# Tianion/topazdb

Hardware: AMD Instinct MI355X
Metric: GiB/s device-resident SSTable block decode+checksum, 4KiB blocks, 1 MI355X (higher is better)
Workload: dtype u8; 1 GPU; 4k: 1048576 blocks/GPU x 4155 B median, 34.0 entries/block, tag 1 (Uncompress); blocks_per_gpu=1048576, input_bytes_per_gpu=4356833280, parallelism=shard1

## Files before the change

### topazdb_amd/csrc/tpz_decode.hip

```cpp

#include <hip/hip_runtime.h>
#include <stdint.h>

#include "tpz_internal.h"
#include "tpz_spill.hip"

namespace tpz {

typedef uint32_t u32;
typedef uint64_t u64;

constexpr int kWave = 64;
#ifdef TPZ_ABL_W20
#ifdef TPZ_ABL_W8
constexpr int kWavesPerWG = 8;
#else
constexpr int kWavesPerWG = 10;
#endif
#else
constexpr int kWavesPerWG = 16;
#endif
constexpr int kWGThreads = kWave * kWavesPerWG;
constexpr u32 kRowShift = 4, kRowBlocks = 1u << kRowShift;
#ifndef TPZ_ROW_AHEAD
#define TPZ_ROW_AHEAD 3
#endif
constexpr u32 kRowAhead = TPZ_ROW_AHEAD, kRowRing = 16;
constexpr u32 kRowExit = 0xFFFFFFFFu;
constexpr int kTableBytes = kNumCrcTables * 256 * 4;
constexpr int kGuard = 96;

constexpr int kWinRounds = 5;
constexpr int kWinBytes = 4352;
constexpr u32 kWaveMaxLen = kWinBytes - 16;
#ifdef TPZ_ABL_W20
constexpr int kWaveTabBytes = 16 * 1024;
constexpr u32 kWaveMaxN = 63;
constexpr int kWaveTabSlots = 128;
#else
constexpr int kWaveTabBytes = kTableBytes;
constexpr u32 kWaveMaxN = 255;
constexpr int kWaveTabSlots = 512;
#endif
constexpr int kWaveMapLen = 288;
constexpr int kSlotBytes = kGuard + kWinBytes + 32 + kWaveTabSlots * 4 + 2 * kWaveMapLen;
static_assert(kSlotBytes % 16 == 0 && kWaveMapLen % 8 == 0, "slot alignment");
static_assert(2 * kWaveMaxN + 1 <= (u32)kWaveTabSlots, "entry table");
constexpr int kWaveLds = kWaveTabBytes + kWavesPerWG * kSlotBytes;
static_assert(kWaveLds <= 163840, "wave path LDS");

constexpr int kBigWaves = 16;
constexpr int kBigThreads = kBigWaves * kWave;
constexpr int kBigWinBytes = 94208;
constexpr u32 kBigMaxLen = TPZ_LDS_BLOCK_BYTES;
constexpr int kBigMapLen = 5904;
constexpr int kBigStage = (kBigWinBytes + 16 * kBigThreads - 1) / (16 * kBigThreads);
constexpr int kBigMaxGroups = 736;
constexpr int kBigMaxWin = 96;
constexpr int kBigLdsSlots = 960;
constexpr int kBigSuper = 20;
constexpr int kBigLds = kTableBytes + kGuard + kBigWinBytes + 32 + kBigMapLen * 2 +
                        kBigMaxGroups * 10 + kBigMaxWin * 4 + kBigWaves * 4 + kBigLdsSlots * 8;
static_assert(kBigMaxLen + 16 <= kBigWinBytes, "big window");
static_assert(kBigMapLen % 8 == 0 && (kWaveMaxLen + 2) / 16 + 3 <= (u32)kWaveMapLen &&
              (kBigMaxLen + 2) / 16 + 3 <= (u32)kBigMapLen, "map sizes");
static_assert(kBigLds <= 163840, "big path LDS");
static_assert((kTableBytes + kGuard + kBigWinBytes + 32 + kBigMapLen * 2 + kBigMaxWin * 4 +
               kBigWaves * 4) % 8 == 0, "big path entry table alignment");

__device__ __forceinline__ u32 lane_id() {
  u32 l = __builtin_amdgcn_mbcnt_hi(~0u, __builtin_amdgcn_mbcnt_lo(~0u, 0u));
  asm volatile("" : "+v"(l));
  return l;
}
__device__ __forceinline__ u32 uni(u32 x) { return __builtin_amdgcn_readfirstlane(x); }
__device__ __forceinline__ u64 uni64(u64 x) {
  u32 lo = __builtin_amdgcn_readfirstlane((u32)x), hi = __builtin_amdgcn_readfirstlane((u32)(x >> 32));
  return ((u64)hi << 32) | lo;
}
__device__ __forceinline__ u32 readlane(u32 x, int l) { return __builtin_amdgcn_readlane(x, l); }
template <int CTRL>
__device__ __forceinline__ u32 dpp(u32 x) {
  return (u32)__builtin_amdgcn_update_dpp(0, (int)x, CTRL, 0xF, 0xF, true);
}
constexpr int kRowShr = 0x110;
constexpr int kRowShl = 0x100;

__device__ __forceinline__ u32 lds_u32(const uint8_t* base, u32 a) {
  const u32* p = reinterpret_cast<const u32*>(base + (a & ~3u));
  return __builtin_amdgcn_alignbyte(p[1], p[0], a & 3u);
}
__device__ __forceinline__ u32 lds_be16(const uint8_t* base, u32 a) {
  u32 w = lds_u32(base, a);
  return ((w & 0xFFu) << 8) | ((w >> 8) & 0xFFu);
}
__device__ __forceinline__ u32 bswap32(u32 w) { return __builtin_bswap32(w); }

__device__ __forceinline__ uint4 lds_window16(const uint8_t* base, int x) {
  typedef u32 u32x2 __attribute__((ext_vector_type(2)));
  const u32x2* p = reinterpret_cast<const u32x2*>(base + (x & ~7));
  u32x2 a = p[0], b = p[1], c = p[2];
  asm volatile("" : "+v"(a), "+v"(b), "+v"(c));
  const u32 s = (u32)x & 3u;
  const bool h = ((u32)x & 4u) != 0;
  const u32 s0 = h ? a.y : a.x, s1 = h ? b.x : a.y, s2 = h ? b.y : b.x, s3 = h ? c.x : b.y,
            s4 = h ? c.y : c.x;
  return make_uint4(__builtin_amdgcn_alignbyte(s1, s0, s), __builtin_amdgcn_alignbyte(s2, s1, s),
                    __builtin_amdgcn_alignbyte(s3, s2, s), __builtin_amdgcn_alignbyte(s4, s3, s));
}

#ifdef TPZ_ABL_NOCF
__device__ __forceinline__ u32 tlook(const u32* tab, int id, u32 byte) {
  u32 z = byte;
  asm volatile("" : "+v"(z));
  return tab[id * 256 + (((z & 0x10000u) + __builtin_amdgcn_mbcnt_lo(~0u, 0u)) & 31u)];
}
#elif defined(TPZ_ABL_W20)
__device__ __forceinline__ u32 tlook(const u32* tab, int id, u32 byte) { return tab[(id & 15) * 256 + byte]; }
#else
__device__ __forceinline__ u32 tlook(const u32* tab, int id, u32 byte) { return tab[id * 256 + byte]; }
#endif

__device__ __forceinline__ u32 xor3(u32 a, u32 b, u32 c) { return __builtin_amdgcn_bitop3_b32(a, b, c, 0x96); }

__device__ __forceinline__ u32 slice16(const u32* tab, u32 w0, u32 w1, u32 w2, u32 w3) {
  u32 c = xor3(tlook(tab, 15, w0 & 0xFF), tlook(tab, 14, (w0 >> 8) & 0xFF), tlook(tab, 13, (w0 >> 16) & 0xFF));
  c = xor3(c, tlook(tab, 12, w0 >> 24), tlook(tab, 11, w1 & 0xFF));
  c = xor3(c, tlook(tab, 10, (w1 >> 8) & 0xFF), tlook(tab, 9, (w1 >> 16) & 0xFF));
  c = xor3(c, tlook(tab, 8, w1 >> 24), tlook(tab, 7, w2 & 0xFF));
  c = xor3(c, tlook(tab, 6, (w2 >> 8) & 0xFF), tlook(tab, 5, (w2 >> 16) & 0xFF));
  c = xor3(c, tlook(tab, 4, w2 >> 24), tlook(tab, 3, w3 & 0xFF));
  c = xor3(c, tlook(tab, 2, (w3 >> 8) & 0xFF), tlook(tab, 1, (w3 >> 16) & 0xFF));
  return c ^ tlook(tab, 0, w3 >> 24);
}

__device__ __forceinline__ u32 crc_shift_small(const u32* tab, u32 a, u32 k) {
  u32 r = k >= 4 ? 0u : (a >> (8 * k));
  for (u32 i = 0; i < 4 && i < k; i++) r ^= tlook(tab, (int)(k - 1 - i), (a >> (8 * i)) & 0xFF);
  return r;
}

__device__ __forceinline__ u32 crc_unshift_small(const u32* tab, u32 r, u32 k) {
#ifdef TPZ_ABL_W20
  return r;
#endif
  for (u32 i = 0; i < k; i++) {
    const u32 b = tlook(tab, kCrcInvTable, r >> 24);
    r = ((r ^ tlook(tab, 0, b)) << 8) | b;
  }
  return r;
}

__device__ __forceinline__ u32 gf_mul(u32 a, u32 b) {
  u32 p = 0;
#pragma unroll
  for (int i = 0; i < 32; i++) {
    p ^= (a & (0x80000000u >> i)) ? b : 0u;
    b = (b >> 1) ^ ((b & 1u) ? 0xEDB88320u : 0u);
  }
  return p;
}

__device__ __forceinline__ u32 gf_mul_lane(u32 a, u32 b) {
  u32 p = 0;
#pragma unroll
  for (int i = 0; i < 32; i++) {
    const u32 m = (u32)((int)(a << i) >> 31);
    p ^= b & m;
    b = (b >> 1) ^ (0xEDB88320u & (u32)(-(int)(b & 1u)));
  }
  return p;
}

__device__ __forceinline__ u32 wave_xor(u32 x) {
  x ^= (u32)__builtin_amdgcn_update_dpp(0, (int)x, 0x100 + 1, 0xF, 0xF, true);
  x ^= (u32)__builtin_amdgcn_update_dpp(0, (int)x, 0x100 + 2, 0xF, 0xF, true);
  x ^= (u32)__builtin_amdgcn_update_dpp(0, (int)x, 0x100 + 4, 0xF, 0xF, true);
  x ^= (u32)__builtin_amdgcn_update_dpp(0, (int)x, 0x100 + 8, 0xF, 0xF, true);
  return __builtin_amdgcn_readlane(x, 0) ^ __builtin_amdgcn_readlane(x, 16) ^
         __builtin_amdgcn_readlane(x, 32) ^ __builtin_amdgcn_readlane(x, 48);
}

template <int J>
__device__ __forceinline__ u32 crc_shift(const u32* tab, u32 a) {
  constexpr int b0 = 16 + 4 * J;
  return xor3(tlook(tab, b0, a & 0xFF), tlook(tab, b0 + 1, (a >> 8) & 0xFF),
              tlook(tab, b0 + 2, (a >> 16) & 0xFF)) ^ tlook(tab, b0 + 3, a >> 24);
}

__device__ __forceinline__ uint4 keep_head(uint4 v, u32 k) {
  const u64 lo = (u64)v.y << 32 | v.x, hi = (u64)v.w << 32 | v.z;
  const u64 mlo = k >= 8 ? ~0ull : ((1ull << (8 * k)) - 1);
  const u64 mhi = k >= 16 ? ~0ull : (k <= 8 ? 0ull : ((1ull << (8 * (k - 8))) - 1));
  const u64 a = lo & mlo, b = hi & mhi;
  return make_uint4((u32)a, (u32)(a >> 32), (u32)b, (u32)(b >> 32));
}

__device__ __forceinline__ uint4 zero_head(uint4 v, u32 k) {
  const u64 lo = (u64)v.y << 32 | v.x, hi = (u64)v.w << 32 | v.z;
  const u64 mlo = k >= 8 ? 0ull : (~0ull << (8 * k));
// ... 487 lines not shown
    j++;
    e0 = e1, d0 = d1, e1 = e2, d1 = d2, e2 = e3, d2 = d3;
  }
  const bool b1 = act && j + 1 < F.nk && e0 < x0 + 16;
  const bool b2 = b1 && j + 2 < F.nk && e1 < x0 + 16;
  uint4 acc = src(act ? (int)x0 + d0 : -kGuard);
  const uint4 n1 = src(b1 ? (int)x0 + d1 : -kGuard);
  const uint4 n2 = src(b2 ? (int)x0 + d2 : -kGuard);
  const bool rw = __ballot(act && (e0 <= x0 || (b2 && e2 < x0 + 16 && j + 3 < F.nk))) != 0;
  if (rw) rare |= 1u << w;
  if (b1) acc = merge_at(acc, n1, (int)(e0 - x0));
  if (b2) acc = merge_at(acc, n2, (int)(e1 - x0));
  if (FLAT)
    D.put(c, acc, rw);
  else
    __builtin_amdgcn_raw_buffer_store_b128(__builtin_bit_cast(__attribute__((ext_vector_type(4))) u32, acc),
                                           F.out, rw ? kOob : x0, 0, 0);
  return carry_out;
}

template <bool SHORT, bool FLAT, class S>
__device__ __forceinline__ u32 copy_crc_fused(const u32* tab, const S& src, const ColSmall& col,
                                              const uint16_t* map, u32 nk, u32 tot, uint8_t* dst,
                                              const FlatOut& D, const uint8_t* win, int pb, u32 Pa,
                                              u32 kshift, Stamps& St, u32 w3, const Out& o,
                                              PendingCrc& pd) {
  const u32 lane = lane_id();
  FastWin F;
  F.nk = nk;
  F.tot = tot;
  F.nch = (tot + 15) >> 4;
  F.npad = FLAT ? F.nch : (F.nch + 7) & ~7u;
  F.last = nk ? nk - 1 : 0u;
  F.out = __builtin_amdgcn_make_buffer_rsrc(dst, (short)0, FLAT ? 0 : (int)(F.npad * 16), 0x00020000);
  const u32 nw = (F.npad + 63) >> 6;
  CrcLane L;
  L.seg = (int)Pa - kCrcLaneBytes * (int)(lane + 1);
  L.act = L.seg + kCrcLaneBytes > 0;
  L.c = 0;
  u32 carry = 0, rare = 0, cw[5];
  const bool pl = pd.live != 0;
  u32 cA = pd.lc, want = 0;
  CombLv cl{0u, 0u, 0u, 0u};
  if (pl) {
    cl = comb_issue<0>(tab, cA);
    want = crc_shift_small(tab, ~pd.stored, pd.k);
  }
#pragma unroll
  for (int t = 0; t < 4; t++) {
    cw[t] = carry;
    crc_step(tab, win, pb, L, t);
    carry = (SHORT && (u32)t < w3) ? copy_fast3<FLAT>(src, col, map, F, D, (u32)t, carry, rare)
                                   : copy_fast<FLAT>(src, col, map, F, D, (u32)t, carry, rare);
    if (pl) {
      if (t == 0) { cA = comb_use<0>(cA, cl); cl = comb_issue<1>(tab, cA); }
      if (t == 1) { cA = comb_use<1>(cA, cl); cl = comb_issue<2>(tab, cA); }
      if (t == 2) { cA = comb_use<2>(cA, cl); cl = comb_issue<3>(tab, cA); }
      if (t == 3) { cA = comb_use<3>(cA, cl); cl = comb_issue<4>(tab, cA); }
    }
  }
  cw[4] = carry;
  crc_step(tab, win, pb, L, 4);
  if (pl) {
    cA = comb_use<4>(cA, cl);
    cl = comb_issue<5>(tab, cA);
  }
  if (nw > 4)
    carry = (SHORT && 4u < w3) ? copy_fast3<FLAT>(src, col, map, F, D, 4u, carry, rare)
                               : copy_fast<FLAT>(src, col, map, F, D, 4u, carry, rare);
  if (pl) comb_finish(tab, o, pd, comb_use<5>(cA, cl), want);
  TPZ_STAMP(St, 4);
#ifdef TPZ_ABL_STAMPS
  St.rare += __builtin_popcount(rare);
#endif
  if (rare) {
    for (u32 w = 0; w < nw; w++)
      if (rare & (1u << w)) {
        if (FLAT)
          copy_window(src, col, map, nk, F.tot, FlatDst{&D}, (u32)kWaveMapLen, w, cw[w]);
        else
          copy_window(src, col, map, nk, F.tot, SlotDst{dst, F.npad, F.tot}, (u32)kWaveMapLen, w, cw[w]);
      }
  }
  return crc_lane_value(tab, L);
}

typedef u32 u32x2v __attribute__((ext_vector_type(2)));
typedef u32 u32x4v __attribute__((ext_vector_type(4)));
struct Gath {
  u32 d0, d1, d2, d3, d4;
};
__device__ __forceinline__ Gath gath_issue(const uint8_t* base, int x) {
  const u32* p = reinterpret_cast<const u32*>(base + (x & ~3));
  Gath g;
  g.d0 = p[0];
  g.d1 = p[1];
  g.d2 = p[2];
  g.d3 = p[3];
  g.d4 = p[4];
  return g;
}
__device__ __forceinline__ uint4 gath_finish(Gath g, int x) {
  asm volatile("" : "+v"(g.d0), "+v"(g.d1), "+v"(g.d2), "+v"(g.d3), "+v"(g.d4));
  const u32 s = (u32)x & 3u;
  return make_uint4(__builtin_amdgcn_alignbyte(g.d1, g.d0, s), __builtin_amdgcn_alignbyte(g.d2, g.d1, s),
                    __builtin_amdgcn_alignbyte(g.d3, g.d2, s), __builtin_amdgcn_alignbyte(g.d4, g.d3, s));
}
struct Look16 {
  u32 r[16];
};
__device__ __forceinline__ Look16 look_issue(const u32* tab, u32x4v w, u32 c) {
  Look16 L;
  const u32 w0 = w.x ^ c;
#pragma unroll
  for (int i = 0; i < 4; i++) {
    L.r[i] = tlook(tab, 15 - i, (w0 >> (8 * i)) & 0xFF);
    L.r[4 + i] = tlook(tab, 11 - i, (w.y >> (8 * i)) & 0xFF);
    L.r[8 + i] = tlook(tab, 7 - i, (w.z >> (8 * i)) & 0xFF);
    L.r[12 + i] = tlook(tab, 3 - i, (w.w >> (8 * i)) & 0xFF);
  }
  return L;
}
__device__ __forceinline__ u32 look_xor(const Look16& L) {
  u32 c = xor3(L.r[0], L.r[1], L.r[2]);
  c = xor3(c, L.r[3], L.r[4]);
  c = xor3(c, L.r[5], L.r[6]);
  c = xor3(c, L.r[7], L.r[8]);
  c = xor3(c, L.r[9], L.r[10]);
  c = xor3(c, L.r[11], L.r[12]);
  c = xor3(c, L.r[13], L.r[14]);
  return c ^ L.r[15];
}
#define TPZ_SB() __builtin_amdgcn_sched_barrier(0)

struct PWin {
  u32 m, j;
  u32 e0, e1;
  int d0, d1;
  bool act, cross;
  Gath ga, gn;
};
struct PWin3 {
  u32 e2, e3;
  int d2, d3;
  bool b2;
  Gath g2;
};

struct RegGeom {
  u32 n, KL, VL, db;
};
constexpr u32 kRegShift = 26;
__device__ __forceinline__ u32 reg_recip(u32 d) {
  u32 m = (u32)(__builtin_amdgcn_rcpf((float)d) * (float)(1u << kRegShift)) + 2u;
  asm volatile("" : "+v"(m));
  return uni(m);
}
__device__ __forceinline__ u32 mul24(u32 a, u32 b) { return (a & 0xFFFFFFu) * (b & 0xFFFFFFu); }
__device__ __forceinline__ u32 reg_div(u32 y, u32 m) {
  const u64 p = (u64)(y & 0x1FFFu) * (u64)(m & 0x7FFFFFu);
  return __builtin_amdgcn_alignbit((u32)(p >> 32), (u32)p, kRegShift) & 0x3FFu;
}

template <bool FLAT, u32 K3, bool REG = false>
__device__ __forceinline__ u32 copy_crc_piped(const u32* tab, const ColSmall& col,
                                              const uint16_t* map, u32 nk, u32 tot, uint8_t* dst,
                                              const FlatOut& D, const uint8_t* win, int pb, u32 Pa,
                                              const Out& o, PendingCrc& pd, u32 k3n = K3,
                                              const RegGeom G = RegGeom{0u, 0u, 0u, 0u}) {
  static_assert(!REG || (K3 == 0 && !FLAT), "the regular copy: slotted, no short keys");
  const u32 lane = lane_id();
  FastWin F;
  F.nk = nk;
  F.tot = tot;
  F.nch = (tot + 15) >> 4;
  F.npad = FLAT ? F.nch : (F.nch + 7) & ~7u;
  F.last = nk ? nk - 1 : 0u;
  F.out = __builtin_amdgcn_make_buffer_rsrc(dst, (short)0, FLAT ? 0 : (int)(F.npad * 16), 0x00020000);
  const u32 nw = (F.npad + 63) >> 6;
  const int seg = (int)Pa - kCrcLaneBytes * (int)(lane + 1);
  const bool cact = seg + kCrcLaneBytes > 0;
  const int cbase = cact ? pb + seg : -kGuard;
  auto dread = [&](int t) -> u32x4v {
    return *reinterpret_cast<const u32x4v*>(win + cbase + 16 * t);
  };
  PWin W[4];
  PWin3 W3;
  const u32 r_kc = G.n * G.KL, r_vs = (r_kc + 15) & ~15u, r_S = 4 + G.KL + G.VL;
  const u32 r_mk = REG ? reg_recip(G.KL) : 0u, r_mv = REG ? reg_recip(G.VL) : 0u;
  const int r_gap = (int)(2 + G.KL) - (int)r_vs - (int)((G.n - 1) * (4 + G.VL));
  auto reg_entry = [&](PWin& P, u32 x0, bool isk) {
    const u32 L = isk ? G.KL : G.VL, base = isk ? 0u : r_vs, T = r_S - L;
    const u32 j = reg_div(x0 - base, isk ? r_mk : r_mv);
    const bool last = j + 1 == G.n;
    P.j = 0;
    P.e0 = (!isk && last) ? 0xFFFFu : base + mul24(j + 1, L);
    P.d0 = (int)((isk ? G.db + 2 : G.db + 4 + G.KL - r_vs) + mul24(j, T));
    P.d1 = P.d0 + ((isk && last) ? r_gap : (int)T);
  };
  auto reg_index = [&](PWin& P, u32 w) {
    const u32 x0 = 16 * (64 * w + lane);
    if (1024 * (w + 1) <= r_kc) reg_entry(P, x0, true);
    else if (1024 * w >= r_vs) reg_entry(P, x0, false);
    else reg_entry(P, x0, x0 < r_kc);
    asm volatile("" : "+v"(P.e0), "+v"(P.d0), "+v"(P.d1));
  };
#pragma unroll
  for (int w = 0; w < 4; w++) {
    const u32 c = 64 * w + lane;
    W[w].act = c < F.nch;
    if (!REG) W[w].m = map[min(c, (u32)kWaveMapLen - 1)];
  }
  u32x4v dA = dread(0);
  u32 cA = pd.lc;
  CombLv cl = comb_issue<0>(tab, cA);
  const u32 want = crc_shift_small(tab, ~pd.stored, pd.k);
  TPZ_SB();
  u32 cw[5];
  cw[0] = 0;
  if (REG) {
#pragma unroll
    for (int w = 0; w < 4; w++) reg_index(W[w], (u32)w);
  } else {
#pragma unroll
    for (int w = 0; w < 4; w++) W[w].j = wave_scan_max(W[w].act ? W[w].m : 0u);
#pragma unroll
    for (int w = 0; w < 4; w++) {
      W[w].j = max(W[w].j, cw[w]);
      cw[w + 1] = readlane(W[w].j, 63);
    }
#pragma unroll
    for (int w = 0; w < 4; w++) col.get2(min(W[w].j, F.last), W[w].e0, W[w].d0, W[w].e1, W[w].d1);
  }
  if (K3) col.get2(min(W[0].j + 2, F.last), W3.e2, W3.d2, W3.e3, W3.d3);
  cA = comb_use<0>(cA, cl);
  cl = comb_issue<1>(tab, cA);
  TPZ_SB();
  Look16 LK = look_issue(tab, dA, 0u);
  u32x4v dB = dread(1);
  cA = comb_use<1>(cA, cl);
  cl = comb_issue<2>(tab, cA);
  TPZ_SB();
  u32 rare = 0;
  auto gissue = [&](PWin& P, u32 w) {
    const u32 x0 = 16 * (64 * w + lane);
    if (w < K3 && w < k3n) {
      if (w > 0) col.get2(min(P.j + 2, F.last), W3.e2, W3.d2, W3.e3, W3.d3);
      if (P.act && P.e0 <= x0) {
        P.j++;
        P.e0 = P.e1, P.d0 = P.d1, P.e1 = W3.e2, P.d1 = W3.d2, W3.e2 = W3.e3, W3.d2 = W3.d3;
      }
      P.cross = P.act && P.j + 1 < F.nk && P.e0 < x0 + 16;
      W3.b2 = P.cross && P.j + 2 < F.nk && P.e1 < x0 + 16;
      if (__ballot(P.act && (P.e0 <= x0 || (W3.b2 && W3.e2 < x0 + 16 && P.j + 3 < F.nk))) != 0)
        rare |= 1u << w;
      W3.g2 = gath_issue(win, W3.b2 ? (int)x0 + W3.d2 : -kGuard);
    } else {
      P.cross = P.act && P.j + 1 < F.nk && P.e0 < x0 + 16;
    }
    P.ga = gath_issue(win, P.act ? (int)x0 + P.d0 : -kGuard);
    P.gn = gath_issue(win, P.cross ? (int)x0 + P.d1 : -kGuard);
  };
  auto finish = [&](PWin& P, u32 w) {
    const u32 c = 64 * w + lane;
    const u32 x0 = 16 * c;
    const bool rw = w < K3 && w < k3n && (rare & (1u << w));
    uint4 acc = gath_finish(P.ga, P.act ? (int)x0 + P.d0 : -kGuard);
    const uint4 nx = gath_finish(P.gn, P.cross ? (int)x0 + P.d1 : -kGuard);
    if (P.cross) acc = merge_at(acc, nx, (int)(P.e0 - x0));
    if (w < K3 && w < k3n) {
      const uint4 n2 = gath_finish(W3.g2, W3.b2 ? (int)x0 + W3.d2 : -kGuard);
      if (W3.b2) acc = merge_at(acc, n2, (int)(P.e1 - x0));
    }
    if (FLAT)
      D.put(c, acc, rw);
    else
      __builtin_amdgcn_raw_buffer_store_b128(__builtin_bit_cast(u32x4v, acc), F.out, rw ? kOob : x0, 0, 0);
  };
  gissue(W[0], 0);
  cA = comb_use<2>(cA, cl);
  cl = comb_issue<3>(tab, cA);
  TPZ_SB();
  u32 crc = 0;
  crc = look_xor(LK);
  LK = look_issue(tab, dB, crc);
  dA = dread(2);
  cA = comb_use<3>(cA, cl);
  cl = comb_issue<4>(tab, cA);
  TPZ_SB();
  finish(W[0], 0);
  gissue(W[1], 1);
  cA = comb_use<4>(cA, cl);
  cl = comb_issue<5>(tab, cA);
  TPZ_SB();
  crc = look_xor(LK);
  LK = look_issue(tab, dA, crc);
  dB = dread(3);
  cA = comb_use<5>(cA, cl);
  comb_finish(tab, o, pd, cA, want);
  TPZ_SB();
  finish(W[1], 1);
  gissue(W[2], 2);
  TPZ_SB();
  crc = look_xor(LK);
  LK = look_issue(tab, dB, crc);
  dA = dread(4);
  TPZ_SB();
  finish(W[2], 2);
  gissue(W[3], 3);
  TPZ_SB();
  crc = look_xor(LK);
  LK = look_issue(tab, dA, crc);
  TPZ_SB();
  finish(W[3], 3);
  TPZ_SB();
  crc = look_xor(LK);
  if (nw > 4) {
    if (REG) {
      W[0].act = 256 + lane < F.nch;
      reg_index(W[0], 4u);
      gissue(W[0], 4u);
      finish(W[0], 4u);
    } else {
      (void)copy_fast<FLAT>(Src16{win}, col, map, F, D, 4u, cw[4], rare);
    }
  }
  if (!REG && rare) {
    for (u32 w = 0; w < nw; w++)
      if (rare & (1u << w)) {
        if (FLAT)
          copy_window(Src16{win}, col, map, nk, F.tot, FlatDst{&D}, (u32)kWaveMapLen, w, cw[w]);
        else
          copy_window(Src16{win}, col, map, nk, F.tot, SlotDst{dst, F.npad, F.tot}, (u32)kWaveMapLen, w, cw[w]);
      }
  }
  return crc;
}


__device__ __forceinline__ u32 crc_prepare(uint8_t* win, u32 a0, u32 P) {
  const u32 lane = lane_id();
  const u32 k = ((a0 + P + 15) & ~15u) - (a0 + P);
  if (lane < 4) win[a0 + lane] ^= 0xFFu;
  if (lane < 16) win[a0 + P + lane] = 0;
  __builtin_amdgcn_wave_barrier();
  return k;
}

template <class Col, class MapT, int kMapLen, bool BIG, bool FLAT = false>
__device__ __forceinline__ void decode_block(const u32* tab, uint8_t* win, const Col& col,
                                             MapT* map, u32 a0, u32 len, u32 b, u64 ext_b,
                                             const Out& o, u32 kshift, Stamps& S, PendingCrc& pd,
                                             u64 kf = 0, u64 vf = 0, u64 ef = 0,
                                             const Out* o_lds = nullptr) {
  const u32 lane = lane_id();
  const u32 tag = win[(int)(a0 + len) - 1];
  const u32 stored = bswap32(lds_u32(win, len >= 5 ? a0 + len - 5 : a0));
  const u32 n = lds_be16(win, a0);
  const u32 dk = (u32)kf & 15u, dv = (u32)vf & 15u;
  u32 e_off = 0, e_kl = 0;
  bool e_ok = false;
  if (!BIG) {
    e_off = lds_be16(win, a0 + 2 + 2 * lane);
    const u32 Pn = len - 5, db0 = a0 + 2 + 2 * n;
    e_ok = len >= 7 && lane < n && Pn >= 2 + 2 * n && e_off + 2 <= Pn - 2 - 2 * n;
    e_kl = lds_be16(win, e_ok ? db0 + e_off : a0);
  }
  if (pd.early) finish_pending(tab, o, pd);
  FinishAtExit fin{tab, o, pd, true};
  if (len == 0) { put_meta(o, b, TPZ_BLOCK_EMPTY, 0, 0); return; }
  if (tag == 0 || tag > 3) { put_meta(o, b, TPZ_BLOCK_BAD_TAG, 0, 0); return; }
  if (tag != 1) { put_meta(o, b, TPZ_BLOCK_UNSUPPORTED_CODEC, 0, 0); return; }
  if (len - 1 < 4) { put_meta(o, b, TPZ_BLOCK_MALFORMED, 0, 0); return; }
  const u32 P = len - 5;
  const int pb = (int)a0;
  u32 st = TPZ_BLOCK_OK, cnt = n;
  bool fuse = false;
  bool f_short = false;
  u32 f_w3 = 0;
  u32 f_nk = 0, f_tot = 0;
  uint8_t* f_dst = nullptr;
  FlatOut fo;
  if (P < 2 || P < 2 + 2 * n) {
    st = TPZ_BLOCK_MALFORMED;
    cnt = 0;
  } else if (!BIG && n > kWaveMaxN) {
    const Out& oc = o_lds ? *o_lds : o;
    if (FLAT) defer_to(oc.spill_list, oc.spill_count, b);
    else defer_to(oc.defer_list, oc.defer_count, b);
    return;
  } else {
    const u32 db = a0 + 2 + 2 * n;
    const u32 dl = P - 2 - 2 * n;
    const bool slots_fit = FLAT || 6u * n <= len;
    uint2* ends_g = reinterpret_cast<uint2*>(o.ends) + uni64((FLAT || o.efirst) ? ef : entry_base(ext_b, b));
    const u32 n_pad = o.efirst ? n : (n + 15) & ~15u;
    u32 r_vl = 0;
    bool r_ok = false;
    if constexpr (!BIG && !FLAT) {
      r_ok = e_ok && e_off + 4 + e_kl <= dl;
      if (r_ok) { r_vl = lds_be16(win, db + e_off + 2 + e_kl); r_ok = e_off + 4 + e_kl + r_vl <= dl; }
      const u32 KL = readlane(e_kl, 0), VL = readlane(r_vl, 0), es = 4 + KL + VL;
      bool reg = n != 0 && KL >= 16 && VL >= 16 && P >= 4 && slots_fit &&
                 !__ballot(lane < n && !(r_ok && e_off == mul24(lane, es) && e_kl == KL && r_vl == VL));
      for (u32 g0 = 64; reg && g0 < n; g0 += 64) {
        const u32 i = g0 + lane;
        bool same = true;
        if (i < n) {
          const u32 off = lds_be16(win, a0 + 2 + 2 * i);
          same = off == mul24(i, es) && off + 4 + KL + VL <= dl;
          if (same) same = lds_be16(win, db + off) == KL && lds_be16(win, db + off + 2 + KL) == VL;
        }
        reg = !__ballot(!same);
      }
      const u32 kc = n * KL, vc = n * VL, vs = stream_vstart<false>(kc, 0u, 0u);
      if (reg && vs + vc <= len + 2u) {
        for (u32 g0 = 0; g0 < n; g0 += 64) {
          const u32 i = g0 + lane;
          __builtin_amdgcn_raw_buffer_store_b64(
              __builtin_bit_cast(__attribute__((ext_vector_type(2))) u32,
                                 i < n ? make_uint2(mul24(i + 1, KL), mul24(i + 1, VL)) : make_uint2(0, 0)),
              whole_rsrc(ends_g), i < n_pad ? 8 * i : kOob, 0, 0);
        }
        TPZ_STAMP(S, 2);
        TPZ_STAMP(S, 3);
        __builtin_amdgcn_wave_barrier();
        const u32 k = crc_prepare(win, a0, P);
        fin.on = false;
        const u32 lc = copy_crc_piped<false, 0u, true>(
            tab, *reinterpret_cast<const ColSmall*>(&col), reinterpret_cast<const uint16_t*>(map),
            2 * n, vs + vc, o.data + slot_base(ext_b, b), fo, win, pb, P + k, o, pd, 0u,
            RegGeom{n, KL, VL, db});
        pd = PendingCrc{1u, b, st, cnt, stored, k, lc, 0u};
        return;
      }
    }
    {
      constexpr u32 per = 16 / sizeof(MapT);
      const u32 nz = min((u32)kMapLen, ((len >> 4) + 3 + per - 1) / per * per);
      for (u32 i = lane; i < nz / per; i += 64)
        reinterpret_cast<uint4*>(map)[i] = make_uint4(0, 0, 0, 0);
    }
    u32 ktot = 0, knz_all = 0;
    if (n > 64) {
      for (u32 g0 = 0; g0 < n; g0 += 64) {
        const u32 i = g0 + lane;
        u32 kl = 0;
        if (i < n) {
          const u32 off = lds_be16(win, a0 + 2 + 2 * i);
          if (off + 2 <= dl) {
            kl = lds_be16(win, db + off);
            if (off + 4 + kl > dl) kl = 0;
          }
        }
        knz_all += __builtin_popcountll(__ballot(kl != 0));
        ktot += readlane(wave_scan_incl(kl), 63);
      }
    }
    u32 kc = 0, vc = 0, knz = 0, vnz = 0;
    bool bad = false, short_k = false, short_v = false;
    for (u32 g0 = 0; g0 < n; g0 += 64) {
      const u32 i = g0 + lane;
      const bool act = i < n;
      u32 off = 0, kl = 0, vl = 0;
      bool ok = true;
      if (act) {
        if (!BIG && !FLAT && g0 == 0) {
          off = e_off;
          kl = e_kl;
          vl = r_vl;
          ok = r_ok;
        } else {
          if (!BIG && g0 == 0) {
            off = e_off;
            ok = e_ok;
            if (ok) { kl = e_kl; ok = off + 4 + kl <= dl; }
          } else {
            off = lds_be16(win, a0 + 2 + 2 * i);
            ok = off + 2 <= dl;
            if (ok) { kl = lds_be16(win, db + off); ok = off + 4 + kl <= dl; }
          }
          if (ok) { vl = lds_be16(win, db + off + 2 + kl); ok = off + 4 + kl + vl <= dl; }
        }
        if (!ok) kl = vl = 0;
      }
      bad |= __ballot(act && !ok) != 0;
      short_k |= __ballot(kl != 0 && kl < 16) != 0;
      short_v |= __ballot(vl != 0 && vl < 16) != 0;
      const u32 ki = wave_scan_incl(kl) + kc;
      const u32 vi = wave_scan_incl(vl) + vc;
      const u64 kmask = __ballot(kl != 0), vmask = __ballot(vl != 0);
      if (n <= 64) {
        ktot = readlane(ki, 63);
        knz_all = __builtin_popcountll(kmask);
      }
      const u32 vs = stream_vstart<FLAT>(ktot, dk, dv);
      __builtin_amdgcn_raw_buffer_store_b64(
          __builtin_bit_cast(__attribute__((ext_vector_type(2))) u32,
                             act ? make_uint2(ki, vi) : make_uint2(0, 0)),
          whole_rsrc(ends_g), (slots_fit && i < n_pad) ? 8 * i : kOob, 0, 0);
      if (act && slots_fit) {
        if (kl) {
          const u32 m = knz + lanes_below(kmask);
          const u32 ke = ki + dk;
          col.put(m, ke, (int)(db + off + 2) - (int)(ke - kl));
          if (((ke + 15) >> 4) < (u32)kMapLen) map[(ke + 15) >> 4] = (MapT)(m + 1);
        }
        if (vl) {
          const u32 m = knz_all + vnz + lanes_below(vmask);
          const u32 ve = vs + vi;
          col.put(m, ve, (int)(db + off + 4 + kl) - (int)(ve - vl));
          if (((ve + 15) >> 4) < (u32)kMapLen) map[(ve + 15) >> 4] = (MapT)(m + 1);
        }
      }
      knz += __builtin_popcountll(kmask);
      vnz += __builtin_popcountll(vmask);
      kc = readlane(ki, 63);
      vc = readlane(vi, 63);
    }

    const u32 vs = stream_vstart<FLAT>(kc, dk, dv);
    TPZ_STAMP(S, 2);
    if (bad || !slots_fit || vs + vc > len + (FLAT ? 47u : 2u)) {
      const Out& oc = o_lds ? *o_lds : o;
      defer_to(oc.spill_list, oc.spill_count, b);
      return;
    } else {
      if (BIG) {
        asm volatile("s_waitcnt vmcnt(0)" ::: "memory");
        __builtin_amdgcn_fence(__ATOMIC_RELEASE, "workgroup");
      }
      __builtin_amdgcn_wave_barrier();
      const u32 tot = FLAT ? (vc ? vs + vc : (kc ? dk + kc : 0u)) : vs + vc;
#ifndef TPZ_ABL_NOCOPY
#if !defined(TPZ_ABL_NOCRC) && !defined(TPZ_ABL_MEMONLY)
#ifdef TPZ_ABL_UNFUSED
      if (false) {
#else
      if (!BIG && P >= 4) {
#endif
        fuse = true;
        f_w3 = short_v ? 5u : (short_k ? (((FLAT ? dk : 0u) + kc + 15) / 16 + 63) / 64 : 0u);
        f_short = f_w3 != 0;
        f_nk = knz + vnz;
        f_tot = tot;
        f_dst = FLAT ? nullptr : o.data + slot_base(ext_b, b);
        if (FLAT) fo = flat_out(o, kf, vf, kc, vc);
      } else
#endif
      if (FLAT) {
        fo = flat_out(o, kf, vf, kc, vc);
        copy_stream(Src16{win}, col, map, knz + vnz, tot, FlatDst{&fo}, (u32)kMapLen);
      } else {
        const u32 nch = (tot + 15) >> 4;
        copy_stream(Src16{win}, col, map, knz + vnz, tot,
                    SlotDst{o.data + slot_base(ext_b, b), (nch + 7) & ~7u, tot}, (u32)kMapLen);
      }
#endif
    }
    TPZ_STAMP(S, 3);
  }
  __builtin_amdgcn_wave_barrier();
  u32 crc;
  if (P >= 4) {
    const u32 k = crc_prepare(win, a0, P);
#if defined(TPZ_ABL_NOCRC) || defined(TPZ_ABL_MEMONLY)
    crc = stored;
#else
    u32 R;
    if (!BIG && fuse) {
      u32 lc;
      fin.on = false;
      if (!f_short) {
        lc = copy_crc_piped<FLAT, 0u>(tab, *reinterpret_cast<const ColSmall*>(&col),
                                         reinterpret_cast<const uint16_t*>(map), f_nk, f_tot, f_dst,
                                         fo, win, pb, P + k, o, pd);
      } else if (f_w3 <= 2u) {
        lc = copy_crc_piped<FLAT, 2u>(tab, *reinterpret_cast<const ColSmall*>(&col),
                                      reinterpret_cast<const uint16_t*>(map), f_nk, f_tot, f_dst,
                                      fo, win, pb, P + k, o, pd, FLAT ? 2u : f_w3);
        f_short = false;
      } else
      {
        lc = f_short
          ? copy_crc_fused<true, FLAT>(tab, Src16{win}, *reinterpret_cast<const ColSmall*>(&col),
                                       reinterpret_cast<const uint16_t*>(map), f_nk, f_tot, f_dst,
                                       fo, win, pb, P + k, kshift, S, f_w3, o, pd)
          : copy_crc_fused<false, FLAT>(tab, Src16{win}, *reinterpret_cast<const ColSmall*>(&col),
// ... 146 lines not shown
#else
  const u32 cshift = CS;
#endif
  const u32 kChunk = 1u << cshift, rshift = kRowShift - cshift;
  u32 pend_slot = ~0u, pend_row = 0;
  const u32 kq = 1u << rshift;
  auto publish = [&]() {
    if (pend_slot != ~0u) {
      if (lane == 0) {

        if ((u64)pend_row * kRowBlocks >= p.n_blocks) {
          __hip_atomic_store(&claims_done, 1u, __ATOMIC_RELAXED, __HIP_MEMORY_SCOPE_WORKGROUP);
          const u32 Q = __hip_atomic_fetch_add(&chunk_next, 0u, __ATOMIC_RELAXED,
                                               __HIP_MEMORY_SCOPE_WORKGROUP);
          atomicMin(&exit_slot, Q == 0 ? kRowAhead : (Q - 1) / kq + kRowAhead + 1);
        }
        __hip_atomic_store(&row_ent[pend_slot % kRowRing], (u64)pend_row | (u64)pend_slot << 32,
                           __ATOMIC_RELAXED, __HIP_MEMORY_SCOPE_WORKGROUP);
      }
      pend_slot = ~0u;
    }
  };
  const bool dyn_rows = rshift != 0;
  u32 q_tk = 0;
  if (lane == 0) q_tk = atomicAdd(&chunk_next, 1u);
  auto claim_chunk = [&]() -> u32 {
    for (;;) {
      publish();
      const u32 q_old = q_tk;
      if (lane == 0) q_tk = atomicAdd(&chunk_next, 1u);
      const u32 q = uni(q_old);
      if (!dyn_rows) {
        const u64 f = ((u64)q * gridDim.x + blockIdx.x) * kRowBlocks;
        return f < p.n_blocks ? (u32)f : p.n_blocks;
      }
      const u32 slot_q = q >> rshift;
      if (slot_q >= uni(__hip_atomic_load(&exit_slot, __ATOMIC_RELAXED, __HIP_MEMORY_SCOPE_WORKGROUP)))
        return p.n_blocks;
      if ((q & ((1u << rshift) - 1u)) == 0) {
#ifdef TPZ_ABL_ROWLATE
        rowlate_delay(p, wid, 0);
#endif
        if (!uni(__hip_atomic_load(&claims_done, __ATOMIC_RELAXED, __HIP_MEMORY_SCOPE_WORKGROUP))) {
          pend_slot = slot_q + kRowAhead;
#ifdef TPZ_ABL_ROWLATE
          rowlate_delay(p, wid, 1);
#endif
          if (lane == 0) pend_row = atomicAdd(p.row_ctr, 1u);
        } else if (lane == 0) {
          const u32 sx = slot_q + kRowAhead;
          __hip_atomic_store(&row_ent[sx % kRowRing], (u64)kRowExit | (u64)sx << 32, __ATOMIC_RELAXED,
                             __HIP_MEMORY_SCOPE_WORKGROUP);
        }
      }
      u32 row = 0;
      if (lane == 0) {
        u32 spins = 0;
        u64 ent;
        while ((u32)((ent = __hip_atomic_load(&row_ent[slot_q % kRowRing], __ATOMIC_RELAXED,
                                              __HIP_MEMORY_SCOPE_WORKGROUP)) >> 32) != slot_q) {
          const u32 rs = (u32)(ent >> 32);
          if (rs != ~0u && (int)(rs - slot_q) > 0) {
            atomicOr(p.err, 4u);
            break;
          }
          __builtin_amdgcn_s_sleep(2);
          if (++spins == (1u << 22)) {
            atomicOr(p.err, 2u);
            break;
          }
        }
        row = (u32)(ent >> 32) != slot_q ? kRowExit : (u32)ent;
      }
      row = uni(row);
      if (row != kRowExit) {
        const u64 f = (u64)row * kRowBlocks + ((q & ((1u << rshift) - 1u)) << cshift);
        if (f < p.n_blocks) return (u32)f;
      }
    }
  };
  auto chunk_first = [](u32 f) -> u32 { return f; };
  u64 gs_cur, gs_nxt;
  auto load_group = [&](u32 q, u64& gs) {
#ifdef TPZ_ABL_ONCHIP
    u32 bb = (chunk_first(q) & kOnchipMask) + (lane <= kChunk ? lane : 0u);
#else
    u32 bb = chunk_first(q) + (lane <= kChunk ? lane : 0u);
#endif
    bb = bb < p.n_blocks ? bb : p.n_blocks;
    gs = p.ext[bb];
  };
  auto lane64 = [](u64 x, u32 l) { return ((u64)readlane((u32)(x >> 32), l) << 32) | readlane((u32)x, l); };
  auto triage_group = [&](u32 q, u64 gs) {
    const u32 glo = (u32)__builtin_amdgcn_update_dpp((int)readlane((u32)gs, 16), (int)(u32)gs,
                                                     kRowShl + 1, 0xF, 0xF, false);
    const u32 ghi = (u32)__builtin_amdgcn_update_dpp((int)readlane((u32)(gs >> 32), 16),
                                                     (int)(u32)(gs >> 32), kRowShl + 1, 0xF, 0xF, false);
    const u64 ge = ((u64)ghi << 32) | glo;
    const u32 cf = chunk_first(q), bb = cf + lane;
    const bool lng = lane < kChunk && lane < p.n_blocks - cf && ge - gs > kWaveMaxLen;
    if (!__ballot(lng)) return;
    const Out& oc = out_lds;
    u32 nent = 0xFFFFu;
    if (lng) nent = ((u32)p.src[gs] << 8) | p.src[gs + 1];
    const bool to_bw = lng && nent < 64 && oc.bw_list && ge - gs <= TPZ_BIGWAVE_BLOCK_BYTES;
    const bool to_spill = lng && !to_bw && (FLAT || ge - gs > kBigMaxLen);
    if (oc.bw_list) defer_lanes(oc.bw_list, oc.bw_count, to_bw, (u32)bb);
    defer_lanes(oc.spill_list, oc.spill_count, to_spill, (u32)bb);
    defer_lanes(oc.defer_list, oc.defer_count, lng && !to_bw && !to_spill, (u32)bb);
  };
  u32 q_cur = claim_chunk(), q_nxt = claim_chunk();
  load_group(q_cur, gs_cur);
  load_group(q_nxt, gs_nxt);
  triage_group(q_cur, gs_cur);
  u32 j = 0;
  u32 b = chunk_first(q_cur);

  uint4 v[kWinRounds];
  u64 s_cur = 0, e_cur = 0;
  u64 kf_cur = 0, vf_cur = 0, ef_cur = 0;
  auto issue = [&](u32 bb, u32 jj, u64& s, u64& e) {
    if (FLAT && bb >= p.n_blocks) return;
    if (bb < p.n_blocks) {
      if (FLAT) {
        kf_cur = const_load(p.out.kfirst, bb);
        vf_cur = const_load(p.out.vfirst, bb);
        ef_cur = const_load(p.out.efirst, bb);
      } else if (p.out.efirst) {
        ef_cur = const_load(p.out.efirst, bb);
      }
    }
    s = lane64(gs_cur, jj);
    e = lane64(gs_cur, jj + 1);
    const bool take = bb < p.n_blocks && e - s <= kWaveMaxLen;
    if (FLAT && !take) return;
    const u64 ws = s & ~15ull;
    const u32 nbytes = (u32)(e - ws);
    const u32 rounds = (nbytes + 1023) >> 10;
    const u64 e16 = (e + 15) & ~(u64)15;
    const u64 lim = !take ? 0 : p.src_bytes < e16 ? p.src_bytes : e16;
    __amdgpu_buffer_rsrc_t rs = window_rsrc(p.src, lim, take ? ws : 0);
#pragma unroll
    for (int r = 0; r < kWinRounds; r++)
      v[r] = __builtin_bit_cast(uint4, __builtin_amdgcn_raw_buffer_load_b128(rs, (u32)(r * 1024 + lane * 16), 0, 0));
    static_assert(kWaveMaxLen + 64 < kOob - 64u * kVmPad, "padding stores stay out of range");
    vm_pad<FLAT ? 0 : kVmPad>(rs);
    if (take && e + 16 > p.src_bytes) {
#pragma unroll
      for (int r = 0; r < kWinRounds; r++)
        if ((u32)r < rounds) fix_tail(v[r], p.src, ws + r * 1024 + lane * 16, p.src_bytes);
    }
  };
  PendingCrc pd{0u, 0u, 0u, 0u, 0u, 0u, 0u};
#ifndef TPZ_ABL_NOPF
  issue(b, 0, s_cur, e_cur);
#endif

  while (b < p.n_blocks) {
#ifdef TPZ_ABL_NOPF
    issue(b, j, s_cur, e_cur);
#endif
    const u64 s = s_cur, e = e_cur;
    const u64 kf = kf_cur, vf = vf_cur, ef = ef_cur;
    const u32 len64 = (e - s) > 0xFFFFFFFFull ? 0xFFFFFFFFu : (u32)(e - s);
    const bool fits = (e - s) <= kWaveMaxLen;
    if (fits) {
#pragma unroll
      for (int r = 0; r < kWinRounds - 1; r++) *reinterpret_cast<uint4*>(win + r * 1024 + lane * 16) = v[r];
      static_assert(kWinBytes == 4 * 1024 + 256, "round 4 fills lanes 0-15");
      if (lane < 16) *reinterpret_cast<uint4*>(win + 4 * 1024 + lane * 16) = v[4];
      if (lane < (u32)(s & 15u)) win[lane] = 0;
    }
    TPZ_STAMP(S, 0);
    const u32 bcur = b;
    if (++j == kChunk) {
      j = 0;
      q_cur = q_nxt;
      gs_cur = gs_nxt;
      q_nxt = claim_chunk();
      load_group(q_nxt, gs_nxt);
      triage_group(q_cur, gs_cur);
    }
    b = chunk_first(q_cur) + j;
    b = b < p.n_blocks ? b : p.n_blocks;
#ifndef TPZ_ABL_NOPF
    issue(b, j, s_cur, e_cur);
#endif
    __builtin_amdgcn_wave_barrier();
    TPZ_STAMP(S, 1);
    if (fits) {
#ifdef TPZ_ABL_ONCHIP
      const u32 bdec = bcur & kOnchipMask;
#else
      const u32 bdec = bcur;
#endif
      decode_block<ColSmall, uint16_t, kWaveMapLen, false, FLAT>(tab, win, col, map, (u32)(s & 15u),
                                                           len64, bdec, s, p.out, kshift, S, pd, kf, vf,
                                                           ef, &out_lds);
    }
    __builtin_amdgcn_wave_barrier();
    TPZ_STAMP(S, 5);
  }
  publish();
  finish_pending(tab, p.out, pd);
#ifdef TPZ_ABL_STAMPS
  const u32 gw = blockIdx.x * kWavesPerWG + wid;
  if (lane == 0 && gw < (u32)kStampWaves)
    for (int k = 0; k < 7; k++) g_stamps[gw * 8 + k] = S.t[k];
  if (lane == 0 && gw < (u32)kStampWaves) g_stamps[gw * 8 + 7] = S.rare;
#endif
}

__device__ __forceinline__ u32 wave_sum(u32 x) { return readlane(wave_scan_incl(x), 63); }
__device__ __forceinline__ u32 wave_max(u32 x) { return readlane(wave_scan_max(x), 63); }

struct GroupSums {
  u32* kb;
  u32* vb;
  uint16_t* cnt;
};

struct BigSums {
  u32 kb = 0, vb = 0, kn = 0, vn = 0;
  bool bad = false;
  __device__ __forceinline__ void add(const GroupSums& gs, u32 lo, u32 hi) {
    const u32 lane = lane_id();
    for (u32 u0 = lo; u0 < hi; u0 += 64) {
      const u32 u = u0 + lane;
      const bool in = u < hi;
      kb += wave_sum(in ? gs.kb[u] : 0u);
      vb += wave_sum(in ? gs.vb[u] : 0u);
      const u32 g = in ? (u32)gs.cnt[u] : 0u;
      const u32 c = wave_sum((g & 0x7Fu) | (((g >> 7) & 0x7Fu) << 16));
      kn += c & 0xFFFFu;
      vn += c >> 16;
      bad |= __ballot((g >> 14) & 1u) != 0;
    }
  }
};

__device__ __forceinline__ void parse_entry(const uint8_t* win, u32 a0, u32 db, u32 dl, u32 i,
                                            u32& off, u32& kl, u32& vl, bool& ok) {
  off = lds_be16(win, a0 + 2 + 2 * i);
  ok = off + 2 <= dl;
  kl = vl = 0;
  if (ok) { kl = lds_be16(win, db + off); ok = off + 4 + kl <= dl; }
  if (ok) { vl = lds_be16(win, db + off + 2 + kl); ok = off + 4 + kl + vl <= dl; }
  if (!ok) kl = vl = 0;
}

__device__ __forceinline__ u32 big_crc_round(const Params& p, const u32* tab, const uint8_t* win,
                                             u32 a0, u32 P, u32 Pa, u32 r) {
  typedef u32 u32x4 __attribute__((ext_vector_type(4)));
  const u32 lane = lane_id();
  const int seg = (int)Pa - 5120 * (int)r - kCrcLaneBytes * (int)(lane + 1);
  u32 c = 0;
  if (seg + kCrcLaneBytes > 0) {
#pragma unroll
    for (int q = 0; q < kCrcLaneBytes / 16; q++) {
      const int base = seg + 16 * q;
      u32x4 w = *reinterpret_cast<const u32x4*>(win + (int)a0 + base);
      if (base < 4 || base + 16 > (int)P) {
        const int zl = (int)P - base, zh = (int)Pa - base;
        w.x = (w.x ^ byte_mask(-base, 4 - base, 0)) & ~byte_mask(zl, zh, 0);
        w.y = (w.y ^ byte_mask(-base, 4 - base, 1)) & ~byte_mask(zl, zh, 1);
        w.z = (w.z ^ byte_mask(-base, 4 - base, 2)) & ~byte_mask(zl, zh, 2);
        w.w = (w.w ^ byte_mask(-base, 4 - base, 3)) & ~byte_mask(zl, zh, 3);
      }
      c = slice16(tab, w.x ^ c, w.y, w.z, w.w);
    }
  }
  return gf_mul(p.xp[r], crc_combine(tab, c));
}

template <class Col, bool kGlobalCol>
__device__ __forceinline__ void big_block(const Params& p, const u32* tab, uint8_t* win,
                                          const Col& col, uint16_t* map, const GroupSums& gsum, u32* wmax,
                                          u32* xs, u32 a0, u32 len, u32 n, u32 stored, u32 b,
                                          u64 ext_b, Stamps& S) {
  const u32 wid = uni(threadIdx.x >> 6), lane = lane_id();
  const Out& o = p.out;
  const u32 P = len - 5;
  const u32 k = ((a0 + P + 15) & ~15u) - (a0 + P);
  const u32 Pa = P + k;
#if defined(TPZ_ABL_NOCRC) || defined(TPZ_ABL_MEMONLY)
  const bool crc_wave = false;
#else
  const bool crc_wave = P >= 4;
#endif
  const u32 Sr = crc_wave ? (Pa + 5119) / 5120 : 0u;
  u32 A = 0;
  for (u32 r = kBigWaves - 1 - wid; r < Sr; r += kBigWaves) A ^= big_crc_round(p, tab, win, a0, P, Pa, r);
  if (lane == 0) xs[wid] = A;
  TPZ_STAMP(S, 4);

  u32 st = TPZ_BLOCK_OK, bcnt = n;
  u32 nk = 0, tot = 0;
  bool copy = false, spill = false;
  if (P < 2 || P < 2 + 2 * n) {
    st = TPZ_BLOCK_MALFORMED;
    bcnt = 0;
    __syncthreads();
  } else {
    const u32 db = a0 + 2 + 2 * n, dl = P - 2 - 2 * n;
    const bool slots_fit = 6u * n <= len;
    uint2* ends_g = reinterpret_cast<uint2*>(o.ends) +
                    uni64(o.efirst ? const_load(o.efirst, b) : entry_base(ext_b, b));
    const u32 n_pad = o.efirst ? n : (n + 15) & ~15u;
    const u32 G = (n + 63) >> 6;
    for (u32 g = wid; g < G; g += kBigWaves) {
      const u32 i = 64 * g + lane;
      u32 off = 0, kl = 0, vl = 0;
      bool ok = true;
      if (i < n) parse_entry(win, a0, db, dl, i, off, kl, vl, ok);
      const u32 kb = wave_sum(kl), vb = wave_sum(vl);
      const u32 kn = __builtin_popcountll(__ballot(kl != 0)), vn = __builtin_popcountll(__ballot(vl != 0));
      const bool bad = __ballot(!ok) != 0;
      if (lane == 0) {
        gsum.kb[g] = kb;
        gsum.vb[g] = vb;
        gsum.cnt[g] = (uint16_t)(kn | (vn << 7) | ((u32)bad << 14));
      }
    }
    if (G > 1) __syncthreads();
    if (wid < G) {
      BigSums T;
      T.add(gsum, 0, G);
      const u32 vs = (T.kb + 15) & ~15u;
      BigSums C;
      u32 done = 0;
      for (u32 g = wid; g < G; g += kBigWaves) {
        C.add(gsum, done, g);
        done = g;
        const u32 i = 64 * g + lane;
        const bool act = i < n;
        u32 off = 0, kl = 0, vl = 0;
        bool ok = true;
        if (act) parse_entry(win, a0, db, dl, i, off, kl, vl, ok);
        const u32 ki = wave_scan_incl(kl) + C.kb;
        const u32 vi = wave_scan_incl(vl) + C.vb;
        const u64 kmask = __ballot(kl != 0), vmask = __ballot(vl != 0);
        __builtin_amdgcn_raw_buffer_store_b64(
            __builtin_bit_cast(__attribute__((ext_vector_type(2))) u32,
                               act ? make_uint2(ki, vi) : make_uint2(0, 0)),
            whole_rsrc(ends_g), (slots_fit && i < n_pad) ? 8 * i : kOob, 0, 0);
        if (act && slots_fit) {
          if (kl) {
            const u32 m = C.kn + lanes_below(kmask);
            col.put(m, ki, (int)(db + off + 2) - (int)(ki - kl));
            if (((ki + 15) >> 4) < (u32)kBigMapLen) map[(ki + 15) >> 4] = (uint16_t)(m + 1);
          }
// ... 297 lines not shown
```

Measured before the change: 2369 GiB/s.

## Cache packed regular-geometry copy indices in LDS across blocks with same shape

For blocks whose keys and values all have uniform lengths, the per-chunk source offsets and cross-boundary split points are precomputed once into a packed 32-bit word per chunk and stored in the wave's LDS entry-table slot. The words are keyed by (n, KL, VL). Later blocks with the same geometry reuse them with a single vector LDS read instead of recomputing reciprocal divisions per chunk. The copy loop's REG path is simplified to unpack these words and issue gathers directly. The cost is a recompute-and-store whenever the geometry changes, plus reliance on the table slot holding the cache undisturbed between blocks. The trailing fifth chunk group is still computed on the fly.

```diff
diff --git a/topazdb_amd/csrc/tpz_decode.hip b/topazdb_amd/csrc/tpz_decode.hip
--- a/topazdb_amd/csrc/tpz_decode.hip
+++ b/topazdb_amd/csrc/tpz_decode.hip
@@ -46,6 +46,7 @@
 constexpr int kSlotBytes = kGuard + kWinBytes + 32 + kWaveTabSlots * 4 + 2 * kWaveMapLen;
 static_assert(kSlotBytes % 16 == 0 && kWaveMapLen % 8 == 0, "slot alignment");
 static_assert(2 * kWaveMaxN + 1 <= (u32)kWaveTabSlots, "entry table");
+static_assert(kWaveTabSlots * 4 + 2 * kWaveMapLen >= kWave * 16, "index cache");
 constexpr int kWaveLds = kWaveTabBytes + kWavesPerWG * kSlotBytes;
 static_assert(kWaveLds <= 163840, "wave path LDS");
 
@@ -839,7 +840,9 @@
 };
 constexpr u32 kRegShift = 26;
 __device__ __forceinline__ u32 reg_recip(u32 d) {
-  u32 m = (u32)(__builtin_amdgcn_rcpf((float)d) * (float)(1u << kRegShift)) + 2u;
+  float f = (float)d;
+  asm volatile("" : "+v"(f));
+  u32 m = (u32)(__builtin_amdgcn_rcpf(f) * (float)(1u << kRegShift)) + 2u;
   asm volatile("" : "+v"(m));
   return uni(m);
 }
@@ -848,13 +851,68 @@
   const u64 p = (u64)(y & 0x1FFFu) * (u64)(m & 0x7FFFFFu);
   return __builtin_amdgcn_alignbit((u32)(p >> 32), (u32)p, kRegShift) & 0x3FFu;
 }
+
+struct RegForm {
+  u32 n, KL, VL, kc, vs, S, mk, mv;
+  int gap;
+  __device__ __forceinline__ RegForm(u32 n_, u32 KL_, u32 VL_) : n(n_), KL(KL_), VL(VL_) {
+    kc = n * KL, vs = (kc + 15) & ~15u, S = 4 + KL + VL;
+    mk = reg_recip(KL), mv = reg_recip(VL);
+    gap = (int)(2 + KL) - (int)vs - (int)((n - 1) * (4 + VL));
+  }
+  __device__ __forceinline__ void entry(u32 x0, u32 db, bool isk, u32& e0, int& d0, int& d1) const {
+    const u32 L = isk ? KL : VL, base = isk ? 0u : vs, T = S - L;
+    const u32 j = reg_div(x0 - base, isk ? mk : mv);
+    const bool last = j + 1 == n;
+    e0 = (!isk && last) ? 0xFFFFu : base + mul24(j + 1, L);
+    d0 = (int)((isk ? db + 2 : db + 4 + KL - vs) + mul24(j, T));
+    d1 = d0 + ((isk && last) ? gap : (int)T);
+  }
+  __device__ __forceinline__ void index(u32 w, u32 lane, u32 db, u32& e0, int& d0, int& d1) const {
+    const u32 x0 = 16 * (64 * w + lane);
+    if (1024 * (w + 1) <= kc) entry(x0, db, true, e0, d0, d1);
+    else if (1024 * w >= vs) entry(x0, db, false, e0, d0, d1);
+    else entry(x0, db, x0 < kc, e0, d0, d1);
+  }
+};
+constexpr u32 kRegBias = 16, kRegNoChunk = 0x80000000u | (16u << 26);
+__device__ __forceinline__ u32 reg_pack(const RegForm& R, u32 w, u32 lane, u32 nch) {
+  const u32 c = 64 * w + lane, x0 = 16 * c;
+  u32 e0;
+  int d0, d1;
+  R.entry(x0, 0u, x0 < R.kc, e0, d0, d1);
+  const bool cross = e0 < x0 + 16;
+  const u32 word = ((x0 + (u32)d0) & 0x1FFFu) |
+                   (cross ? (((x0 + (u32)d1 + kRegBias) & 0x1FFFu) << 13) | ((e0 - x0) << 26) : 16u << 26);
+  return c < nch ? word : kRegNoChunk;
+}
+constexpr u32 kRegNone = 0u;
+__device__ __forceinline__ u32 reg_key(u32 n, u32 KL, u32 VL) {
+  return n == 1 ? 0x80000000u | VL << 13 | KL : n << 24 | VL << 12 | KL;
+}
+template <bool ON>
+struct RegKeyVar {
+  u32 key = kRegNone;
+  __device__ __forceinline__ u32* ptr() { return &key; }
+};
+template <>
+struct RegKeyVar<false> {
+  __device__ __forceinline__ u32* ptr() { return nullptr; }
+};
+template <bool ON>
+struct RegWords {
+  u32x4v v;
+};
+template <>
+struct RegWords<false> {};
 
 template <bool FLAT, u32 K3, bool REG = false>
 __device__ __forceinline__ u32 copy_crc_piped(const u32* tab, const ColSmall& col,
                                               const uint16_t* map, u32 nk, u32 tot, uint8_t* dst,
                                               const FlatOut& D, const uint8_t* win, int pb, u32 Pa,
                                               const Out& o, PendingCrc& pd, u32 k3n = K3,
-                                              const RegGeom G = RegGeom{0u, 0u, 0u, 0u}) {
+                                              const RegGeom G = RegGeom{0u, 0u, 0u, 0u},
+                                              const u32x4v rix = u32x4v{0u, 0u, 0u, 0u}) {
   static_assert(!REG || (K3 == 0 && !FLAT), "the regular copy: slotted, no short keys");
   const u32 lane = lane_id();
   FastWin F;
@@ -873,30 +931,19 @@
   };
   PWin W[4];
   PWin3 W3;
-  const u32 r_kc = G.n * G.KL, r_vs = (r_kc + 15) & ~15u, r_S = 4 + G.KL + G.VL;
-  const u32 r_mk = REG ? reg_recip(G.KL) : 0u, r_mv = REG ? reg_recip(G.VL) : 0u;
-  const int r_gap = (int)(2 + G.KL) - (int)r_vs - (int)((G.n - 1) * (4 + G.VL));
-  auto reg_entry = [&](PWin& P, u32 x0, bool isk) {
-    const u32 L = isk ? G.KL : G.VL, base = isk ? 0u : r_vs, T = r_S - L;
-    const u32 j = reg_div(x0 - base, isk ? r_mk : r_mv);
-    const bool last = j + 1 == G.n;
-    P.j = 0;
-    P.e0 = (!isk && last) ? 0xFFFFu : base + mul24(j + 1, L);
-    P.d0 = (int)((isk ? G.db + 2 : G.db + 4 + G.KL - r_vs) + mul24(j, T));
-    P.d1 = P.d0 + ((isk && last) ? r_gap : (int)T);
-  };
-  auto reg_index = [&](PWin& P, u32 w) {
-    const u32 x0 = 16 * (64 * w + lane);
-    if (1024 * (w + 1) <= r_kc) reg_entry(P, x0, true);
-    else if (1024 * w >= r_vs) reg_entry(P, x0, false);
-    else reg_entry(P, x0, x0 < r_kc);
+  auto reg_unpack = [&](PWin& P, u32 word) {
+    P.e0 = (word >> 26) & 31u;
+    P.d0 = (int)word < 0 ? -kGuard : (int)(G.db + (word & 0x1FFFu));
+    P.d1 = P.e0 < 16 ? (int)(G.db - kRegBias + ((word >> 13) & 0x1FFFu)) : -kGuard;
     asm volatile("" : "+v"(P.e0), "+v"(P.d0), "+v"(P.d1));
   };
+  if constexpr (!REG) {
 #pragma unroll
-  for (int w = 0; w < 4; w++) {
-    const u32 c = 64 * w + lane;
-    W[w].act = c < F.nch;
-    if (!REG) W[w].m = map[min(c, (u32)kWaveMapLen - 1)];
+    for (int w = 0; w < 4; w++) {
+      const u32 c = 64 * w + lane;
+      W[w].act = c < F.nch;
+      W[w].m = map[min(c, (u32)kWaveMapLen - 1)];
+    }
   }
   u32x4v dA = dread(0);
   u32 cA = pd.lc;
@@ -906,8 +953,10 @@
   u32 cw[5];
   cw[0] = 0;
   if (REG) {
-#pragma unroll
-    for (int w = 0; w < 4; w++) reg_index(W[w], (u32)w);
+    reg_unpack(W[0], rix.x);
+    reg_unpack(W[1], rix.y);
+    reg_unpack(W[2], rix.z);
+    reg_unpack(W[3], rix.w);
   } else {
 #pragma unroll
     for (int w = 0; w < 4; w++) W[w].j = wave_scan_max(W[w].act ? W[w].m : 0u);
@@ -930,6 +979,11 @@
   TPZ_SB();
   u32 rare = 0;
   auto gissue = [&](PWin& P, u32 w) {
+    if constexpr (REG) {
+      P.ga = gath_issue(win, P.d0);
+      P.gn = gath_issue(win, P.d1);
+      return;
+    }
     const u32 x0 = 16 * (64 * w + lane);
     if (w < K3 && w < k3n) {
       if (w > 0) col.get2(min(P.j + 2, F.last), W3.e2, W3.d2, W3.e3, W3.d3);
@@ -951,6 +1005,13 @@
   auto finish = [&](PWin& P, u32 w) {
     const u32 c = 64 * w + lane;
     const u32 x0 = 16 * c;
+    if constexpr (REG) {
+      uint4 acc = gath_finish(P.ga, P.d0);
+      const uint4 nx = gath_finish(P.gn, P.d1);
+      if (P.e0 < 16) acc = merge_at(acc, nx, (int)P.e0);
+      __builtin_amdgcn_raw_buffer_store_b128(__builtin_bit_cast(u32x4v, acc), F.out, x0, 0, 0);
+      return;
+    }
     const bool rw = w < K3 && w < k3n && (rare & (1u << w));
     uint4 acc = gath_finish(P.ga, P.act ? (int)x0 + P.d0 : -kGuard);
     const uint4 nx = gath_finish(P.gn, P.cross ? (int)x0 + P.d1 : -kGuard);
@@ -1004,8 +1065,15 @@
   crc = look_xor(LK);
   if (nw > 4) {
     if (REG) {
-      W[0].act = 256 + lane < F.nch;
-      reg_index(W[0], 4u);
+      const RegForm R(G.n, G.KL, G.VL);
+      const u32 x0 = 16 * (256 + lane);
+      u32 e0;
+      int d0, d1;
+      R.index(4u, lane, G.db, e0, d0, d1);
+      const bool act = 256 + lane < F.nch, cross = act && e0 < x0 + 16;
+      W[0].e0 = cross ? e0 - x0 : 16u;
+      W[0].d0 = act ? (int)x0 + d0 : -kGuard;
+      W[0].d1 = cross ? (int)x0 + d1 : -kGuard;
       gissue(W[0], 4u);
       finish(W[0], 4u);
     } else {
@@ -1039,7 +1107,7 @@
                                              MapT* map, u32 a0, u32 len, u32 b, u64 ext_b,
                                              const Out& o, u32 kshift, Stamps& S, PendingCrc& pd,
                                              u64 kf = 0, u64 vf = 0, u64 ef = 0,
-                                             const Out* o_lds = nullptr) {
+                                             const Out* o_lds = nullptr, u32* rk = nullptr) {
   const u32 lane = lane_id();
   const u32 tag = win[(int)(a0 + len) - 1];
   const u32 stored = bswap32(lds_u32(win, len >= 5 ? a0 + len - 5 : a0));
@@ -1053,6 +1121,7 @@
     e_ok = len >= 7 && lane < n && Pn >= 2 + 2 * n && e_off + 2 <= Pn - 2 - 2 * n;
     e_kl = lds_be16(win, e_ok ? db0 + e_off : a0);
   }
+  RegWords<!BIG && !FLAT> rix;
   if (pd.early) finish_pending(tab, o, pd);
   FinishAtExit fin{tab, o, pd, true};
   if (len == 0) { put_meta(o, b, TPZ_BLOCK_EMPTY, 0, 0); return; }
@@ -1111,16 +1180,27 @@
         }
         TPZ_STAMP(S, 2);
         TPZ_STAMP(S, 3);
+        const u32 key = reg_key(n, KL, VL);
+        rix.v = *reinterpret_cast<const u32x4v*>(reinterpret_cast<const uint8_t*>(col.t) + 16 * lane);
+        if (*rk != key) {
+          const RegForm R(n, KL, VL);
+          const u32 nch = (vs + vc + 15) >> 4;
+#pragma nounroll
+          for (u32 w = 0; w < 4; w++) col.t[4 * lane + w] = reg_pack(R, w, lane, nch);
+          rix.v = *reinterpret_cast<const u32x4v*>(reinterpret_cast<const uint8_t*>(col.t) + 16 * lane);
+          *rk = key;
+        }
         __builtin_amdgcn_wave_barrier();
         const u32 k = crc_prepare(win, a0, P);
         fin.on = false;
         const u32 lc = copy_crc_piped<false, 0u, true>(
             tab, *reinterpret_cast<const ColSmall*>(&col), reinterpret_cast<const uint16_t*>(map),
             2 * n, vs + vc, o.data + slot_base(ext_b, b), fo, win, pb, P + k, o, pd, 0u,
-            RegGeom{n, KL, VL, db});
+            RegGeom{n, KL, VL, db}, rix.v);
         pd = PendingCrc{1u, b, st, cnt, stored, k, lc, 0u};
         return;
       }
+      *rk = kRegNone;
     }
     {
       constexpr u32 per = 16 / sizeof(MapT);
@@ -1573,6 +1653,7 @@
     }
   };
   PendingCrc pd{0u, 0u, 0u, 0u, 0u, 0u, 0u};
+  RegKeyVar<!FLAT> rk;
 #ifndef TPZ_ABL_NOPF
   issue(b, 0, s_cur, e_cur);
 #endif
@@ -1617,7 +1698,7 @@
 #endif
       decode_block<ColSmall, uint16_t, kWaveMapLen, false, FLAT>(tab, win, col, map, (u32)(s & 15u),
                                                            len64, bdec, s, p.out, kshift, S, pd, kf, vf,
-                                                           ef, &out_lds);
+                                                           ef, &out_lds, rk.ptr());
     }
     __builtin_amdgcn_wave_barrier();
     TPZ_STAMP(S, 5);
```

New measurement: 2453 GiB/s (median of 6 runs). +3.5%, better.
